# libraz/mygram-db

Hardware: AMD Instinct MI355X
Metric: queries/sec + p50 latency, 10M-doc bigram index, batch=1024 3-term AND (higher is better)
Workload: dtype u32 set algebra + f64 BM25

## Files before the change

mygram-db_amd/csrc/mgx_api.cpp:

```cpp
#include <hip/hip_runtime.h>

#include <dlfcn.h>
#include <pthread.h>

#include <algorithm>
#include <atomic>
#include <chrono>
#include <cmath>
#include <condition_variable>
#include <map>
#include <cstdio>
#include <cstdlib>
#include <cstring>
#include <memory>
#include <mutex>
#include <string>
#include <thread>
#include <tuple>
#include <unordered_map>
#include <vector>

#include "../../include/mygram_gpu.h"
#include "mgx_compile.hpp"
#include "mgx_highlight.hpp"
// ... 1481 lines not shown
    bool on() const { return !plan.queries.empty(); }
    bool requested(uint32_t qi) const { return on() && of_query[qi] >= 0; }
  };
  Documents doc;
  bool fetched = false;
  std::vector<mgx_query_result> h_results;
  std::vector<uint32_t> h_docs;
  std::vector<double> h_scores;
  bool executed = false;
  hipStream_t last_stream = nullptr;
  bool timing = false;
  std::vector<std::pair<hipEvent_t, hipEvent_t>> events;
  uint64_t list_bytes = 0;
};

namespace mgx {

constexpr int kSections = 7;
static std::atomic<uint64_t> g_section_us[kSections];
static const char* const kSectionNames[kSections] = {"queries+leaves", "routes", "table uploads", "result blocks",
                                                      "items", "launch order", "descriptors+items"};
struct SectionTimer {
  static bool On() {
    static const bool on = std::getenv("MGX_TRACE_HOST") != nullptr;
    return on;
  }
  std::chrono::steady_clock::time_point t;
  SectionTimer() { if (On()) t = std::chrono::steady_clock::now(); }
  void Mark(int section) {
    if (!On()) return;
    const auto now = std::chrono::steady_clock::now();
    g_section_us[section] += std::chrono::duration_cast<std::chrono::nanoseconds>(now - t).count();
    t = now;
  }
};

using Group = mgx_batch::Group;
using RouteLaunch = mgx_batch::RouteLaunch;

enum class Route : uint8_t {
  kBlock,
  kWave,
  kWaveLists,
  kFast,
  kCand,
  kMerge,
};

static bool EnvZero(const char* name) { return std::getenv(name) && atoi(std::getenv(name)) == 0; }
struct PathSwitches {
  const bool wave = std::getenv("MGX_FORCE_BLOCK_KERNEL") == nullptr;
  const bool fast = wave && !EnvZero("MGX_FAST_PATH"), cand = wave && !EnvZero("MGX_CAND");
  const bool merge = wave && !EnvZero("MGX_MERGE");
};

struct GroupPlan {
  GroupPlan(uint32_t n_, uint32_t mode)
      : n(n_), score_mode(mode == kModeScore), df_mode(mode == kModeTextDf), page_mode(mode == kModeDocPage) {}
  const uint32_t n;
  const bool score_mode, df_mode, page_mode;
  std::vector<DevQuery> dq;
  std::vector<DevLeaf> leaves;
  std::vector<uint32_t> prog;
  std::vector<DevScoreTerm> score;
  std::vector<uint32_t> expl;
  uint32_t max_limit = 1, max_needed = 1;
  std::vector<Route> route;
  std::vector<DevFastQuery> fastq;
  std::vector<uint64_t> wave_tables;
  std::vector<uint32_t> cand_driver;
  std::vector<DevItem> items;
  std::vector<uint32_t> list_begin, item_begin;
  std::vector<DevItem> block, wave, wave_lists, fast[kFastMaxScore], cand, merge;
  std::vector<uint8_t> has_seed;
};

static int LayOutQueries(mgx_batch* b, Group& g, const std::vector<QuerySpec>& specs, GroupPlan& p) {
  std::vector<DevLeaf>& leaves = p.leaves;
  std::vector<uint32_t>& expl = p.expl;
  p.dq.resize(p.n);
  uint32_t max_leaves = 0, max_lds_leaves = 0, max_score = 0, max_stack = 0, max_instr = 0, max_cap = 64;
  for (uint32_t i = 0; i < p.n; ++i) {
    const QuerySpec& s = specs[g.qids[i]];
    DevQuery& q = p.dq[i];
    std::memset(&q, 0, sizeof(q));
    q.leaf_begin = static_cast<uint32_t>(leaves.size());
    q.n_leaves = static_cast<uint32_t>(s.leaves.size());
    q.prog_begin = static_cast<uint32_t>(p.prog.size());
    q.n_instr = static_cast<uint32_t>(s.prog.size());
    q.score_begin = static_cast<uint32_t>(p.score.size());
    q.n_score = static_cast<uint32_t>(s.score.size());
    q.mode = s.mode;
    q.limit = s.limit;
    q.offset = s.offset;
    q.needed = static_cast<uint32_t>(std::min<uint64_t>(static_cast<uint64_t>(s.offset) + s.limit, 0xFFFFFFFFull));
    uint32_t cap = 64;
    if (s.mode == kModeScore)
      while (cap < q.needed && cap < (1u << 30)) cap <<= 1;
    q.cap = cap;
    q.descending = s.reverse;
    q.stack_depth = s.stack_depth;
    q.out_slot = i;
    q.pat_off = s.pat_off;
    q.pat_len = s.pat_len;
    q.vt_begin = s.vt_begin;
    q.vt_count = static_cast<uint32_t>(s.verify_patterns.size());
    q.fz_distance = s.fz_distance;
    q.vp_begin = s.vp_begin;
    q.k1 = s.k1;
    q.b = s.b;
    q.one_minus_b = 1.0 - s.b;
    q.k1_plus_1 = s.k1 + 1.0;
    q.avgdl_clamped = std::max(s.avgdl, 1.0);
    const uint32_t ebase = static_cast<uint32_t>(expl.size());
    uint32_t n_lds = 0;
    for (size_t li = 0; li < s.leaves.size(); ++li) {
      DevLeaf lf = s.leaves[li];
      if (lf.kind == kLeafExplicit) lf.a += ebase;
      bool resident = lf.kind == kLeafList || lf.kind == kLeafExplicit;
      for (const DevScoreTerm& st : s.score) resident = resident || st.leaf == li;
      lf.lds = resident ? n_lds++ : kNoRow;
      leaves.push_back(lf);
    }
    if (n_lds > kMaxLdsLeaves)
      return Fail(MGX_ERR_NOT_IMPLEMENTED,
                  "query " + std::to_string(g.qids[i]) + ": more than 64 sorted-list / scored operands in one query");
    max_lds_leaves = std::max(max_lds_leaves, n_lds);
    p.prog.insert(p.prog.end(), s.prog.begin(), s.prog.end());
    p.score.insert(p.score.end(), s.score.begin(), s.score.end());
    expl.insert(expl.end(), s.explicit_ids.begin(), s.explicit_ids.end());
    while (expl.size() % 4) expl.push_back(0xFFFFFFFFu);
    max_leaves = std::max(max_leaves, q.n_leaves);
    max_score = std::max(max_score, q.n_score);
    max_stack = std::max(max_stack, q.stack_depth);
    max_instr = std::max(max_instr, q.n_instr);
    max_cap = std::max(max_cap, q.cap);
    p.max_limit = std::max(p.max_limit, q.limit);
    p.max_needed = std::max(p.max_needed, q.needed);
    if (!p.df_mode) b->list_bytes += 4 * s.list_postings;
  }
  g.plan = PlanLds(max_leaves, max_lds_leaves, max_score, max_stack, max_instr, max_cap, p.score_mode || p.df_mode);
  return MGX_OK;
}

static bool ResolveFast(mgx_index* idx, const uint64_t* cond_arena, const QuerySpec& s, const DevQuery& q, DevFastQuery* out) {
  DevFastQuery& f = *out;
  for (uint32_t ins : s.prog) {
    const uint32_t op = ins >> 24, arg = ins & 0xFFFFFFu;
    if (op == kOpCount) {
      if (f.n_ops == 0) return false;
      f.ops[f.n_ops - 1].code |= arg << 8;
      continue;
    }
    const DevLeaf& lf = s.leaves[arg];
    if (f.n_ops == static_cast<uint32_t>(kFastMaxOps) || (op == kOpLoad) != (f.n_ops == 0)) return false;
    FastOp o{};
    uint64_t stride = 0;
    if (lf.kind == kLeafGramBitmap) {
      o.base = reinterpret_cast<uint64_t>(idx->dev.gram_bitmaps + static_cast<uint64_t>(lf.b) * idx->dev.gb_row_stride);
      stride = idx->dev.gb_tile_stride * 8;
    } else if (lf.kind == kLeafFilterBitmap) {
      o.base = static_cast<uint64_t>(lf.b) * idx->dev.fb_row_stride * 8;
      stride = idx->dev.fb_tile_stride * 8;
      o.code |= 16u;
    } else if (lf.kind == kLeafCondBitmap) {
      o.base = reinterpret_cast<uint64_t>(cond_arena + static_cast<uint64_t>(lf.b) * idx->dev.fb_row_stride);
      stride = idx->dev.fb_tile_stride * 8;
    } else {
      return false;
    }
    if (stride > 0xFFFFFFFFull) return false;
    o.tile_stride = static_cast<uint32_t>(stride);
    o.code |= (op == kOpLoad || op == kOpOr) ? kFastOr : op == kOpAnd ? kFastAnd : kFastAndNot;
    f.ops[f.n_ops++] = o;
  }
  if (f.n_ops == 0) return false;
  for (size_t t = 0; t < s.score.size(); ++t) {
    const DevLeaf& lf = s.leaves[s.score[t].leaf];
    if (lf.kind != kLeafGramBitmap) return false;
    FastScore& fs = f.score[t];
    fs.nib = reinterpret_cast<uint64_t>(idx->dev.tfnib + static_cast<uint64_t>(lf.b) * idx->dev.nib_row_stride);
    fs.idf = s.score[t].idf;
    fs.gram = lf.a;
    fs.skip_row = lf.row;
  }
  if (s.reverse != 0) {
    double step = 0.0;
    f.blockmax = GetBlockMax(idx, s.k1, s.b, s.avgdl, &step, &f.blockmax_fine);
    if (f.blockmax) {
      f.bm_tile_stride = idx->n_bitmap_rows * 256u;
      f.bmf_tile_stride = idx->n_fine_rows * 1024u;
      double idf_max = 0.0;
      for (size_t t = 0; t < s.score.size(); ++t) idf_max = std::max(idf_max, s.score[t].idf);
      const double wunit = idf_max > 0.0 ? idf_max * (1.0 + 0x1p-40) / 255.0 : 1.0;
      f.bm_inv_unit = 1.0 / (wunit * step);
      f.bm_wpack = f.bm_w4 = f.bm_cint = 0;
      for (size_t t = 0; t < s.score.size(); ++t) {
        const uint32_t w = static_cast<uint32_t>(std::min(255.0, std::ceil(s.score[t].idf / wunit)));
        if (t < 4) f.bm_wpack |= w << (8 * t); else f.bm_w4 = w;
      }
      for (size_t t = 0; t < s.score.size(); ++t) {
        const DevLeaf& lf = s.leaves[s.score[t].leaf];
        FastScore& fs = f.score[t];
        const uint32_t frow = f.blockmax_fine ? idx->h_fine_map[lf.b] : kNoRow;
        fs.bm_mode = frow != kNoRow ? 2u : 1u;
        fs.bm_off = frow != kNoRow ? frow * 1024u : lf.b * 256u;
      }
    }
  }
  f.n_score = static_cast<uint32_t>(s.score.size());
  f.needed = q.needed;
  f.cap = q.cap;
  f.descending = q.descending;
  f.k1 = q.k1;
  f.b = q.b;
  f.one_minus_b = q.one_minus_b;
  f.k1_plus_1 = q.k1_plus_1;
  f.avgdl_clamped = q.avgdl_clamped;
  return true;
}

static void RouteCandMerge(mgx_batch* b, Group& g, const std::vector<QuerySpec>& specs, const PathSwitches& sw,
                           GroupPlan& p) {
  static const uint64_t kMaxPerTile = std::getenv("MGX_CAND_MAX_PER_TILE") ? static_cast<uint64_t>(atoll(std::getenv("MGX_CAND_MAX_PER_TILE"))) : 64ull;
  const mgx_index* idx = b->idx;
  for (uint32_t i = 0; sw.cand && i < p.n; ++i) {
    const QuerySpec& s = specs[g.qids[i]];
    if (p.route[i] == Route::kFast || !s.flat || s.prog.empty()) continue;
    if (p.score_mode && (!s.fast_score_ok || s.score.empty())) continue;
    bool ok = true, counted = false;
    uint32_t driver = kNoLeaf;
    uint64_t best = ~0ull, longest_list = 0;
    for (size_t pc = 0; ok && pc < s.prog.size(); ++pc) {
      const uint32_t op = s.prog[pc] >> 24, arg = s.prog[pc] & 0xFFFFFFu;
      if (op == kOpCount) {
        counted = true;
        continue;
      }
      if ((op == kOpLoad) != (pc == 0) || (op != kOpLoad && op != kOpAnd && op != kOpAndNot)) { ok = false; break; }
      const DevLeaf& lf = s.leaves[arg];
      if (lf.kind != kLeafList && lf.kind != kLeafGramBitmap && !IsFilterKind(lf.kind)) { ok = false; break; }
      if (lf.kind == kLeafList) longest_list = std::max<uint64_t>(longest_list, idx->h_offsets[lf.a + 1] - idx->h_offsets[lf.a]);
      if (op == kOpAndNot || IsFilterKind(lf.kind) || counted) continue;
      const uint64_t sz = idx->h_offsets[lf.a + 1] - idx->h_offsets[lf.a];
      if (sz < best) {
        best = sz;
        driver = arg;
      }
    }
    if (!ok || driver == kNoLeaf || s.leaves[driver].kind != kLeafList) continue;
    for (uint32_t ins : s.prog)
      if ((ins >> 24) == kOpAndNot && (ins & 0xFFFFFFu) == driver) ok = false;
    if (p.score_mode)
      for (const DevScoreTerm& st : s.score)
        ok = ok && st.leaf != kNoLeaf && (s.leaves[st.leaf].kind == kLeafList || s.leaves[st.leaf].kind == kLeafGramBitmap);
    if (!ok) continue;
    DevQuery& q = p.dq[i];
    const bool long_probe = longest_list > 8 * kMaxPerTile * idx->dev.n_tiles;
    if (best > kMaxPerTile * idx->dev.n_tiles || long_probe) {
      uint32_t staged = 0;
      for (size_t li = 0; li < s.leaves.size(); ++li) staged += li != driver ? 1u : 0u;
      if (!p.score_mode || !sw.merge || staged > kMergeMaxOps || q.cap > 256) continue;
      q.pat_off = driver;
      p.route[i] = Route::kMerge;
      g.merge_leaves = std::max(g.merge_leaves, q.n_leaves);
      g.merge_instr = std::max(g.merge_instr, q.n_instr);
      g.merge_ops = std::max(g.merge_ops, staged);
      g.merge_cap = std::max(g.merge_cap, q.cap);
      continue;
    }
    if (p.cand_driver.empty()) p.cand_driver.assign(p.n, kNoLeaf);
    p.cand_driver[i] = driver;
    p.route[i] = Route::kCand;
    g.cand_leaves = std::max(g.cand_leaves, q.n_leaves);
    g.cand_instr = std::max(g.cand_instr, q.n_instr);
    g.cand_cap = std::max(g.cand_cap, q.cap);
  }
  if (CandLdsBytes(g.cand_leaves, g.cand_instr, p.score_mode ? g.cand_cap : 0) > 150 * 1024) {
    for (Route& r : p.route)
      if (r == Route::kCand) r = Route::kBlock;
    p.cand_driver.clear();
  }
  if (MergeLdsBytes(g.merge_leaves, g.merge_instr, g.merge_ops, g.merge_cap) > 150 * 1024)
    for (Route& r : p.route)
      if (r == Route::kMerge) r = Route::kBlock;
}

static int ChooseRoutes(mgx_batch* b, Group& g, const std::vector<QuerySpec>& specs, const PathSwitches& sw,
                        GroupPlan& p) {
  mgx_index* idx = b->idx;
  p.route.assign(p.n, Route::kBlock);
  if (p.score_mode) {
    uint32_t fcap = 64;
    bool have_params = false;
    double pk1 = 0, pb = 0, pavg = 0;
    for (uint32_t i = 0; sw.fast && i < p.n; ++i) {
      const QuerySpec& s = specs[g.qids[i]];
      if (!s.flat || !s.fast_score_ok || s.score.empty() || s.score.size() > static_cast<size_t>(kFastMaxScore)) continue;
      if (p.dq[i].cap > 128) continue;
      if (have_params && (Bits(s.k1) != Bits(pk1) || Bits(s.b) != Bits(pb) || Bits(s.avgdl) != Bits(pavg))) continue;
      DevFastQuery f{};
      if (!ResolveFast(idx, b->cond_arena, s, p.dq[i], &f)) continue;
      if (!have_params) {
        pk1 = s.k1;
        pb = s.b;
        pavg = s.avgdl;
        have_params = true;
      }
      if (p.fastq.empty()) p.fastq.resize(p.n);
      p.fastq[i] = f;
      p.route[i] = Route::kFast;
      fcap = std::max(fcap, f.cap);
    }
    if (have_params) {
      const double* ktab = GetLengthNormTable(idx, pk1, pb, pavg);
      g.fplan = PlanFast(fcap, ktab);
      if (ktab == nullptr || g.fplan.bytes > 64 * 1024)
        for (Route& r : p.route) r = Route::kBlock;
    }

    uint32_t wl = 0, wsc = 0, wi = 0, wc = 64;
    for (uint32_t i = 0; i < p.n; ++i) {
      if (p.route[i] == Route::kFast) continue;
      const QuerySpec& s = specs[g.qids[i]];
      bool ok = sw.wave && s.wave_ok;
      for (const DevScoreTerm& st : s.score)
        ok = ok && (s.leaves[st.leaf].kind == kLeafGramBitmap || s.leaves[st.leaf].kind == kLeafList);
      if (!ok) continue;
      uint64_t tabs[kWaveScoreSlots] = {0, 0, 0};
      for (size_t t = 0; ok && t < s.score.size(); ++t) {
        const DevLeaf& lf = s.leaves[s.score[t].leaf];
        const uint32_t key = lf.kind == kLeafGramBitmap ? lf.b : 0x80000000u | lf.a;
        tabs[t] = GetContributionTable(idx, key, s.score[t].idf, s.k1, s.b, s.avgdl);
        ok = tabs[t] != 0;
      }
      if (!ok) continue;
      if (p.wave_tables.empty()) p.wave_tables.assign(static_cast<size_t>(p.n) * kWaveScoreSlots, 0);
      for (int t = 0; t < kWaveScoreSlots; ++t) p.wave_tables[static_cast<size_t>(i) * kWaveScoreSlots + t] = tabs[t];
      bool lists = false;
      for (const DevLeaf& lf : s.leaves) lists = lists || lf.kind == kLeafList || lf.kind == kLeafExplicit;
      p.route[i] = lists ? Route::kWaveLists : Route::kWave;
      wl = std::max<uint32_t>(wl, p.dq[i].n_leaves);
      wsc = std::max<uint32_t>(wsc, p.dq[i].n_score);
      wi = std::max<uint32_t>(wi, p.dq[i].n_instr);
      wc = std::max<uint32_t>(wc, p.dq[i].cap);
    }
    g.wplan = PlanWave(wl, wsc, wi, wc, idx->dev.max_doc_len, false);
    g.wplan_lists = PlanWave(wl, wsc, wi, wc, idx->dev.max_doc_len, true);
    if (g.wplan_lists.bytes > 160 * 1024)
      for (Route& r : p.route)
        if (r != Route::kFast) r = Route::kBlock;
  }
  if (p.page_mode || p.df_mode) {
    uint32_t wl = 1, wi = 1;
    bool has_list = false;
// ... 274 lines not shown
    d.wave_tables = g.d_tables.as<uint64_t>();
  }
  if (!p.fastq.empty()) MGX_HIP(Upload(g.d_fast_queries, p.fastq.data(), p.fastq.size()));
  d.fast_queries = g.d_fast_queries.as<DevFastQuery>();
  d.dev_index = b->idx->d_dev_index.as<DevIndex>();
  d.cond_bitmaps = b->cond_arena;
  for (int t = 0; t < kFastMaxScore; ++t) MGX_HIP(MakeRoute(g.fast[t], d, p.fast[t]));
  MGX_HIP(MakeRoute(g.wave_lists, d, p.wave_lists));
  MGX_HIP(MakeRoute(g.cand, d, p.cand));
  MGX_HIP(MakeRoute(g.merge, d, p.merge));
  if (p.page_mode && !p.cand.empty()) {
    std::vector<uint8_t> skip(n, 0);
    for (uint32_t i = 0; i < n; ++i) skip[i] = p.route[i] == Route::kCand ? 1 : 0;
    MGX_HIP(Upload(g.d_cand_skip, skip.data(), skip.size()));
  }
  MGX_HIP(MakeRoute(g.block, d, p.block));
  MGX_HIP(MakeRoute(g.wave, d, p.wave));
  MGX_HIP(Upload(g.d_list_begin, p.list_begin.data(), p.list_begin.size()));
  if (p.page_mode) {
    std::vector<DevItem> pw, pb;
    for (uint32_t i = 0; i < n; ++i)
      if (p.route[i] != Route::kCand && !specs[g.qids[i]].fz_op)
        (p.route[i] == Route::kWave ? pw : pb).push_back(DevItem{i, 0, 0, 0});
    g.n_page_fz = 0;
    for (uint32_t i = 0; i < n; ++i)
      if (specs[g.qids[i]].fz_op) {
        pb.push_back(DevItem{i, 0, 0, 0});
        ++g.n_page_fz;
      }
    MGX_HIP(MakeRoute(g.page_wave, d, pw));
    MGX_HIP(MakeRoute(g.page_block, d, pb));
  }
  return MGX_OK;
}

static int UploadGroup(mgx_batch* b, Group& g, uint32_t mode, const std::vector<QuerySpec>& specs) {
  GroupPlan p(static_cast<uint32_t>(g.qids.size()), mode);
  if (p.n == 0) return MGX_OK;
  const PathSwitches sw;
  SectionTimer sec;
  if (const int rc = LayOutQueries(b, g, specs, p)) return rc;
  sec.Mark(0);
  if (const int rc = ChooseRoutes(b, g, specs, sw, p)) return rc;
  sec.Mark(1);
  if (const int rc = UploadTables(b, g, p, sec)) return rc;
  sec.Mark(3);
  CutItems(b, g, specs, p);
  sec.Mark(4);
  if (const int rc = ScheduleItems(b, g, specs, p)) return rc;
  sec.Mark(5);
  if (const int rc = UploadItems(b, g, specs, p)) return rc;
  sec.Mark(6);
  if (std::getenv("MGX_VERBOSE")) {
    size_t fast_queries = 0;
    for (Route r : p.route) fast_queries += r == Route::kFast ? 1 : 0;
    fprintf(stderr,
            "[mgx] %s group: %u queries; fast path %zu items (%zu queries, lds %u B, ring %u), wave kernel %zu items "
            "(lds %u B, lists %zu), block kernel %zu items (lds %u B), candidate-driven %zu queries, list merge %zu "
            "items\n",
            p.score_mode ? "score" : p.page_mode ? "docid-page" : p.df_mode ? "df" : "bitmap", p.n,
            p.fast[0].size() + p.fast[1].size() + p.fast[2].size() + p.fast[3].size() + p.fast[4].size(), fast_queries,
            g.fplan.bytes, g.fplan.ring, p.wave.size() + p.wave_lists.size(), g.wplan.bytes, p.wave_lists.size(),
            p.block.size(), g.plan.bytes, p.cand.size(), p.merge.size());
  }
  return MGX_OK;
}

static CompileView ViewOf(const mgx_index* idx) {
  CompileView v;
  v.offsets = idx->h_offsets.data();
  v.skip_row = idx->h_skip_row.data();
  v.bm_row = idx->h_bm_row.data();
  v.n_grams = idx->n_grams;
  v.n_docs = idx->dev.n_docs;
  v.first_doc_id = idx->dev.first_doc_id;
  v.has_text = idx->dev.text != nullptr;
  v.can_score = idx->can_score;
  v.n_filter_rows = idx->n_filter_rows;
  v.n_filter_columns = idx->n_filter_columns.load(std::memory_order_acquire);
  v.live_row = idx->live_row.load(std::memory_order_relaxed);
  v.bitmaps_clean = idx->bitmaps_clean.load(std::memory_order_relaxed);
  static const bool pk_general = [] {
    const char* e = std::getenv("MGX_PK_SORT_GENERAL");
    return e != nullptr && e[0] != '\0' && e[0] != '0';
  }();
  v.pk_docid_order = !pk_general && !idx->has_doc_map.load(std::memory_order_acquire) && idx->pk_monotone.load(std::memory_order_acquire) &&
                     idx->pk_shortcut.load(std::memory_order_relaxed);
  return v;
}

static int CompileRange(const CompileView& view, const mgx_query* queries, std::vector<QuerySpec>* specs, uint32_t a, uint32_t b) {
  for (uint32_t i = a; i < b; ++i) {
    (*specs)[i].Clear();
    if (const int rc = CompileQuery(view, queries[i], &(*specs)[i])) return Fail(rc, "query " + std::to_string(i) + ": " + g_last_error);
  }
  return MGX_OK;
}

struct CompilePool {
  std::mutex mu, gate;
  std::condition_variable cv_work, cv_done;
  std::vector<std::thread> helpers;
  const CompileView* view = nullptr;
  const mgx_query* queries = nullptr;
  std::vector<QuerySpec>* specs = nullptr;
  uint32_t next = 0, end = 0, pending = 0;
  int rc = MGX_OK;
  std::string error;
  bool stop = false;
  static constexpr uint32_t kChunk = 64;

  void Run(std::unique_lock<std::mutex>& lock) {
    while (next < end) {
      const uint32_t a = next, b = std::min(end, a + kChunk);
// ... 2840 lines not shown
```

mygram-db_amd/csrc/mgx_internal.hpp:

```cpp
#pragma once

#include <cstdint>

namespace mgx {

constexpr int kBlock = 256;
constexpr int kTileShift = 14;
constexpr uint32_t kTileDocs = 1u << kTileShift;
constexpr int kWordsPerTile = kTileDocs / 64;
constexpr int kMaxTilesPerItem = 64;
constexpr uint32_t kNoRow = 0xFFFFFFFFu;
constexpr uint32_t kMaxLeaves = 192;
constexpr uint32_t kMaxLdsLeaves = 64;
constexpr uint32_t kMaxScoreTerms = 64;
constexpr uint32_t kMaxNeeded = 1024;
constexpr uint32_t kMergeMaxOps = 6;
constexpr uint32_t kMatchBuf = 2048;

enum LeafKind : uint32_t {
  kLeafList = 0,
  kLeafGramBitmap = 1,
  kLeafFilterBitmap = 2,
  kLeafRange = 3,
  kLeafExplicit = 4,
// ... 73 lines not shown
  kModeDocCount = 3,
  kModeDocPage = 4,
};
constexpr uint32_t kMaxDocPage = 16384;

struct DevQuery {
  uint32_t leaf_begin, n_leaves;
  uint32_t prog_begin, n_instr;
  uint32_t score_begin, n_score;
  uint32_t mode;
  uint32_t cap;
  uint32_t needed;
  uint32_t limit, offset;
  uint32_t descending;
  uint32_t stack_depth;
  uint32_t out_slot;
  uint32_t pat_off, pat_len;
  uint32_t vt_begin, vt_count;
  uint32_t fz_distance;
  uint32_t vp_begin;
  double k1, b, one_minus_b, k1_plus_1, avgdl_clamped;
};

constexpr uint32_t kFzBuf = 2048;
constexpr uint32_t kFzLdsBytes = kWordsPerTile * 8 + 16 + kFzBuf * 2;

struct DevIndex {
  const uint64_t* offsets;
  const uint32_t* docids;
  const uint8_t* tf;
  const uint64_t* tf_ovf_pos;
  const uint32_t* tf_ovf_val;
  uint32_t n_tf_ovf;
  const uint32_t* doc_len;
  const uint8_t* dl8;
  const uint8_t* tfnib;
  uint64_t nib_row_stride;
  const uint32_t* skip_row;
  const uint32_t* tile_off;
  const uint64_t* gram_bitmaps;
  uint64_t gb_tile_stride, gb_row_stride;
  const uint64_t* filter_bitmaps;
  uint64_t fb_tile_stride, fb_row_stride;
  const uint8_t* text;
  const uint64_t* text_off;
  uint32_t first_doc_id;
  uint32_t n_docs;
  uint32_t n_tiles;
  uint32_t max_doc_len;
};

constexpr int kFastMaxOps = 8;
constexpr int kFastMaxScore = 5;
constexpr uint32_t kFastPoolTf = 14;
#ifndef MGX_FWAVES
#define MGX_FWAVES 8
#endif
constexpr int kFastBlock = 64 * MGX_FWAVES;
constexpr int kFastWaves = kFastBlock / 64;

enum FastOpKind : uint32_t { kFastOr = 0, kFastAnd = 1, kFastAndNot = 2 };
struct FastOp {
  uint64_t base;
  uint32_t tile_stride;
  uint32_t code;
};
struct FastScore {
  uint64_t nib;
  double idf;
  uint32_t gram, skip_row;
  uint32_t bm_mode, bm_off;
};
struct DevFastQuery {
  uint32_t n_ops, n_score, needed, cap;
  uint32_t descending, pad0;
  uint32_t pad1, pad1b;
  uint32_t bm_wpack, bm_w4;
  uint32_t bm_cint, pad2;
  double bm_inv_unit;
  double k1, b, one_minus_b, k1_plus_1, avgdl_clamped;
  const uint8_t* blockmax;
  const uint8_t* blockmax_fine;
  uint32_t bm_tile_stride, bmf_tile_stride;
  FastOp ops[kFastMaxOps];
  FastScore score[kFastMaxScore];
};
static_assert(sizeof(DevFastQuery) % 8 == 0, "DevFastQuery is read with scalar loads");

struct FastPlan {
  uint32_t ring;
  uint32_t max_cap;
  uint32_t bytes, pad;
  const double* ktab;
};
struct TableJob {
  double idf, k1, b, avgdl;
  uint32_t slot, pad;
};
FastPlan PlanFast(uint32_t max_cap, const double* ktab);
uint32_t FastTableDl(uint32_t max_doc_len);

struct DevItem {
  uint32_t query, tile_begin, n_tiles, list;
};

struct DevCondition {
  uint64_t literal;
  double eq_epsilon;
  uint32_t op, null_matches, never_matches;
  uint32_t row;
};
struct DevCondGroup {
  const uint64_t* values;
  const uint8_t* is_null;
  uint32_t value_class, cond_begin, cond_end, pad;
};
static_assert(sizeof(DevCondition) % 8 == 0 && sizeof(DevCondGroup) % 8 == 0, "read with scalar loads");
constexpr uint32_t kCondWordsPerWave = 8;
constexpr uint32_t kCondBlockWords = kCondWordsPerWave * (kBlock / 64);

struct DevBatch {
  const DevItem* items;
  uint32_t n_items;
  const DevQuery* queries;
  const DevLeaf* leaves;
  const uint32_t* prog;
  const DevScoreTerm* score_terms;
  const uint32_t* explicit_pool;
// ... 82 lines not shown
```

mygram-db_amd/csrc/mgx_kernels.hip:

```cpp
#include <hip/hip_runtime.h>

#include <algorithm>
#include <cstdlib>

#include "mgx_fuzzy.hpp"
#include "mgx_internal.hpp"
#include "mgx_launch.hpp"

namespace mgx {

#ifdef MGX_ABLATION
#define MGX_ABLATE(bt, bit) (((bt).debug_skip & (bit)) != 0)
#else
#define MGX_ABLATE(bt, bit) false
#endif


__device__ __forceinline__ int lane_id() { return threadIdx.x & 63; }

__device__ __forceinline__ uint32_t wave_uniform(uint32_t v) { return __builtin_amdgcn_readfirstlane(v); }
__device__ __forceinline__ float wave_uniform(float v) {
  return __uint_as_float(__builtin_amdgcn_readfirstlane(__float_as_uint(v)));
}
__device__ __forceinline__ uint64_t wave_uniform(uint64_t v) {
// ... 1634 lines not shown
      }
    }
    if (tid == 0) bt.cand_n[it.list] = min(total, q.needed);
  }
}

__global__ __launch_bounds__(kWaveBlock, 6) void wave_score_kernel(DevIndex ix, DevBatch bt, WavePlan plan) {
  wave_score_body(ix, bt, plan);
}
__global__ __launch_bounds__(kWaveBlock, 6) void wave_score_lists_kernel(DevIndex ix, DevBatch bt, WavePlan plan) {
  wave_score_body(ix, bt, plan);
}


#ifndef MGX_FPL
#define MGX_FPL 4
#endif
constexpr int kFastPerLane = MGX_FPL;
constexpr uint32_t kFastRound = 64 * kFastPerLane;
constexpr uint32_t kFastPairs = 320;

struct FastOffsets {
  uint32_t ktab, pairs, ring, tk_keys, tk_docs, misc, total;
};
__host__ __device__ inline FastOffsets carve_fast(const FastPlan& p) {
  FastOffsets o;
  uint32_t at = 0;
  o.ktab = at;     at += 256 * 8;
  o.pairs = at;    at += kFastWaves * kFastPairs * 8;
  o.ring = at;     at += kFastWaves * p.ring * 4;
  o.tk_keys = at;  at += kFastWaves * 2 * p.max_cap * 8;
  o.tk_docs = at;  at += kFastWaves * 2 * p.max_cap * 4;
  o.misc = at;     at += 64;
  o.total = at;
  return o;
}
uint32_t FastTableDl(uint32_t max_doc_len) {
  const uint32_t t = max_doc_len + 1 < kTableDlMax ? max_doc_len + 1 : kTableDlMax;
  return (t + 1u) & ~1u;
}
FastPlan PlanFast(uint32_t max_cap, const double* ktab) {
  FastPlan p{};
  p.ring = kFastRound + 128;
  p.max_cap = max_cap;
  p.ktab = ktab;
  p.bytes = carve_fast(p).total;
  return p;
}

typedef uint32_t u32x4 __attribute__((ext_vector_type(4)));
typedef const u32x4 __attribute__((address_space(1)))* gptr_u4;
typedef const uint32_t __attribute__((address_space(1)))* gptr_u1;
typedef const DevFastQuery __attribute__((address_space(4)))* FastQueryPtr;

__device__ __noinline__ uint32_t fast_exact_tf(const DevIndex* ix, uint32_t gram, uint32_t row, uint32_t slot) {
  return exact_tf(*ix, gram, row, slot);
}

template <int T>
__device__ __forceinline__ void fast_load_blockmax(const FastQueryPtr fq, uint32_t tile, uint32_t lane, u32x4 (&raw)[T]) {
  const uint64_t bm = reinterpret_cast<uint64_t>(fq->blockmax), bmf = reinterpret_cast<uint64_t>(fq->blockmax_fine);
  const uint32_t st = fq->bm_tile_stride, stf = fq->bmf_tile_stride;
#pragma unroll
  for (int i = 0; i < T; ++i) {
    const bool fine = fq->score[i].bm_mode == 2u;
    const uint64_t row = (fine ? bmf : bm) + static_cast<uint64_t>(tile) * (fine ? stf : st) + fq->score[i].bm_off;
    const uint32_t off = fine ? lane << 4 : (lane >> 2) << 4;
    raw[i] = *reinterpret_cast<gptr_u4>(row + off);
  }
}

template <int T>
__device__ __forceinline__ uint32_t fast_quarter_mask(const FastQueryPtr fq, uint32_t lane, const u32x4 (&raw)[T],
                                                      uint64_t bound) {
  const uint32_t tint = static_cast<uint32_t>(
      fmin(floor(key_score(bound, true) * fq->bm_inv_unit * (1.0 - 0x1p-30)), 4294967040.0));
  const uint32_t wpack = fq->bm_wpack, w4 = fq->bm_w4, cint = fq->bm_cint;
  uint32_t bmw[T][4];
#pragma unroll
  for (int i = 0; i < T; ++i) {
    bmw[i][0] = raw[i].x;
    bmw[i][1] = raw[i].y;
    bmw[i][2] = raw[i].z;
    bmw[i][3] = raw[i].w;
    const uint32_t mode = fq->score[i].bm_mode;
    if (mode == 1u) {
      const uint32_t l3 = lane & 3u;
      const uint32_t c = l3 == 0u ? raw[i].x : l3 == 1u ? raw[i].y : l3 == 2u ? raw[i].z : raw[i].w;
      bmw[i][0] = __builtin_amdgcn_perm(0u, c, 0x00000000u);
      bmw[i][1] = __builtin_amdgcn_perm(0u, c, 0x01010101u);
      bmw[i][2] = __builtin_amdgcn_perm(0u, c, 0x02020202u);
      bmw[i][3] = __builtin_amdgcn_perm(0u, c, 0x03030303u);
    } else if (mode != 2u) {
      bmw[i][0] = bmw[i][1] = bmw[i][2] = bmw[i][3] = 0;
    }
  }
  uint32_t mk = 0;
#pragma unroll
  for (int k = 0; k < 4; ++k) {
    const uint32_t t0 = bmw[0][k], t1 = T > 1 ? bmw[T > 1 ? 1 : 0][k] : 0u, t2 = T > 2 ? bmw[T > 2 ? 2 : 0][k] : 0u,
                   t3 = T > 3 ? bmw[T > 3 ? 3 : 0][k] : 0u;
    const uint32_t lo01 = __builtin_amdgcn_perm(t1, t0, 0x05010400u), hi01 = __builtin_amdgcn_perm(t1, t0, 0x07030602u);
    const uint32_t lo23 = T > 2 ? __builtin_amdgcn_perm(t3, t2, 0x05010400u) : 0u;
    const uint32_t hi23 = T > 2 ? __builtin_amdgcn_perm(t3, t2, 0x07030602u) : 0u;
    uint32_t qb[4];
    qb[0] = __builtin_amdgcn_perm(lo23, lo01, 0x05040100u);
    qb[1] = __builtin_amdgcn_perm(lo23, lo01, 0x07060302u);
    qb[2] = __builtin_amdgcn_perm(hi23, hi01, 0x05040100u);
    qb[3] = __builtin_amdgcn_perm(hi23, hi01, 0x07060302u);
#pragma unroll
    for (int j = 0; j < 4; ++j) {
      uint32_t ub = __builtin_amdgcn_udot4(qb[j], wpack, cint, false);
      if (T > 4) ub += w4 * ((bmw[T > 4 ? 4 : 0][k] >> (8 * j)) & 255u);
      if (ub >= tint) mk |= 1u << (4 * k + j);
    }
  }
  return mk;
}

template <int T>
__device__ __noinline__ uint32_t fast_remask(const FastQueryPtr fq, uint32_t tile, uint32_t lane, uint64_t bound) {
  u32x4 raw[T];
  fast_load_blockmax<T>(fq, tile, lane, raw);
  return fast_quarter_mask<T>(fq, lane, raw, bound);
}

template <int T>
__device__ __forceinline__ void bitmap_score_body(const DevIndex& ix, const DevBatch& bt, const FastPlan& plan,
                                                  const FastQueryPtr fq, const DevItem it) {
  extern __shared__ __attribute__((aligned(16))) unsigned char smem[];
  const FastOffsets fo = carve_fast(plan);
  const uint32_t tid = threadIdx.x, lane = tid & 63u, wave = wave_uniform(tid >> 6);
  double* const ktab = reinterpret_cast<double*>(smem + fo.ktab);
  uint32_t* const ring = reinterpret_cast<uint32_t*>(smem + fo.ring) + wave * plan.ring;
  uint2* const pairs = reinterpret_cast<uint2*>(smem + fo.pairs) + wave * kFastPairs;
  uint32_t* const misc = reinterpret_cast<uint32_t*>(smem + fo.misc);
  const uint32_t n_ops = fq->n_ops;
  const bool desc = fq->descending != 0;
  const uint32_t tile_begin = it.tile_begin;
  const uint32_t tile_end = min(tile_begin + it.n_tiles, ix.n_tiles);

  if (tid < 256) ktab[tid] = plan.ktab[tid];

  WaveTopK tk;
  tk.cap = fq->cap;
  tk.needed = fq->needed;
  tk.lds_sort = true;
  tk.keys = reinterpret_cast<uint64_t*>(smem + fo.tk_keys) + static_cast<size_t>(wave) * 2 * fq->cap;
  tk.docs = reinterpret_cast<uint32_t*>(smem + fo.tk_docs) + static_cast<size_t>(wave) * 2 * fq->cap;
  tk.have = 0;
  tk.pend = 0;
  tk.bound_key = 0;
  tk.bound_doc = 0;
  tk.gbound_ptr = bt.bounds ? bt.bounds + it.query : nullptr;
  tk.gbound = 0;
  for (uint32_t i = lane; i < 2 * tk.cap; i += 64) {
    tk.keys[i] = 0;
    tk.docs[i] = 0;
  }
  __syncthreads();

  __amdgpu_buffer_rsrc_t nib_rsrc[T];
  double idf[T];
#pragma unroll
  for (int i = 0; i < T; ++i) {
    nib_rsrc[i] = __builtin_amdgcn_make_buffer_rsrc(reinterpret_cast<void*>(fq->score[i].nib), 0,
                                                    static_cast<int>((ix.n_docs + 1u) >> 1), 0x00020000);
    idf[i] = fq->score[i].idf;
  }
  const __amdgpu_buffer_rsrc_t dl_rsrc = __builtin_amdgcn_make_buffer_rsrc(
      const_cast<uint8_t*>(ix.dl8), 0, static_cast<int>(ix.n_docs), 0x00020000);
  const double k1_plus_1 = fq->k1_plus_1;
  const bool prune = fq->blockmax != 0;

  uint32_t cnt0 = 0, cnt1 = 0, cnt2 = 0, cnt3 = 0, cnt_res = 0;
  uint32_t pend = 0;
  uint32_t np = 0;

  auto score_round = [&](uint32_t g0, uint32_t n) {
    uint32_t slot[kFastPerLane], dli[kFastPerLane], nb[kFastPerLane][T];
#pragma unroll
    for (int m = 0; m < kFastPerLane; ++m) {
// ... 10 lines not shown
    for (int m = 0; m < kFastPerLane; ++m) {
      if (static_cast<uint32_t>(m) * 64u >= n) break;
      uint32_t sl = slot[0], dl = dli[0], nbm[T];
#pragma unroll
      for (int i = 0; i < T; ++i) nbm[i] = nb[0][i];
#pragma unroll
      for (int mm = 1; mm < kFastPerLane; ++mm) {
        if (m == mm) {
          sl = slot[mm];
          dl = dli[mm];
#pragma unroll
          for (int i = 0; i < T; ++i) nbm[i] = nb[mm][i];
        }
      }
      const bool valid = static_cast<uint32_t>(m) * 64u + lane < n;
      double kd = ktab[dl];
      const uint32_t sh = (sl & 1u) << 2;
      uint32_t tf[T], mx = 0;
#pragma unroll
      for (int i = 0; i < T; ++i) {
        tf[i] = (nbm[i] >> sh) & 15u;
        mx = max(mx, tf[i]);
      }
      if (__ballot(valid && (mx == 15u || dl == 255u)) != 0) {
#pragma unroll
        for (int i = 0; i < T; ++i)
          if (valid && tf[i] == 15u) tf[i] = fast_exact_tf(bt.dev_index, fq->score[i].gram, fq->score[i].skip_row, sl);
        if (valid && dl == 255u) {
          const double dld = static_cast<double>(ix.doc_len[sl]);
          kd = fq->k1 * (fq->one_minus_b + fq->b * dld / fq->avgdl_clamped);
        }
      }
      double score = 0.0;
#pragma unroll
      for (int i = 0; i < T; ++i) {
        const double tfd = static_cast<double>(tf[i]);
        const double c = tf[i] != 0u ? idf[i] * (tfd * k1_plus_1) / (tfd + kd) : 0.0;
        score = i == 0 ? c : score + c;
      }
      const uint32_t doc = ix.first_doc_id + sl;
      wave_topk_offer(tk, valid, score_key(score, desc), desc ? doc : ~doc);
    }
  };

  auto load_half = [&](uint32_t o, uint32_t tile, uint32_t h) {
    const uint64_t op_base = fq->ops[o].base;
    const uint32_t op_code = fq->ops[o].code, op_stride = fq->ops[o].tile_stride;
    const uint64_t base = op_base + ((op_code & 16u) ? reinterpret_cast<uint64_t>(ix.filter_bitmaps) : 0ull) +
                          static_cast<uint64_t>(tile) * op_stride;
    const gptr_u4 p = reinterpret_cast<gptr_u4>(base) + lane * 2 + h;
    return p[0];
  };

  for (uint32_t tile = tile_begin + wave;; tile += kFastWaves) {
    const bool flush = tile >= tile_end;
    uint32_t a[8] = {0, 0, 0, 0, 0, 0, 0, 0};
    uint64_t bound = 0;
    if (!flush) {
      wave_topk_refresh_gbound(tk);
      uint32_t qmask = 0xFFFFu;
      if (prune) {
        bound = tk.gbound;
        if (tk.have >= tk.needed && tk.bound_key > bound) bound = tk.bound_key;
      }
      u32x4 raw[T];
#pragma unroll
      for (int i = 0; i < T; ++i) raw[i] = u32x4{0u, 0u, 0u, 0u};
      if (prune) fast_load_blockmax<T>(fq, tile, lane, raw);
      auto combine = [&](int h, uint32_t o, const u32x4 w) {
        const uint32_t code = fq->ops[o].code;
        const uint32_t x[4] = {w.x, w.y, w.z, w.w};
        const uint32_t kind = wave_uniform(code & 15u);
        if (kind == kFastAnd) {
#pragma unroll
          for (int j = 0; j < 4; ++j) a[h * 4 + j] &= x[j];
        } else if (kind == kFastOr) {
#pragma unroll
          for (int j = 0; j < 4; ++j) a[h * 4 + j] |= x[j];
        } else {
#pragma unroll
          for (int j = 0; j < 4; ++j) a[h * 4 + j] &= ~x[j];
        }
        const uint32_t cmask = wave_uniform(code >> 8);
        if (cmask) {
          uint32_t pc = 0;
#pragma unroll
          for (int j = 0; j < 4; ++j) pc += __popc(a[h * 4 + j]);
          if (cmask & 1u) cnt0 += pc;
          if (cmask & 2u) cnt1 += pc;
          if (cmask & 4u) cnt2 += pc;
          if (cmask & 8u) cnt3 += pc;
        }
      };
      const uint32_t o1 = min(1u, n_ops - 1u), o2 = min(2u, n_ops - 1u);
      u32x4 w[2][3];
#pragma unroll
      for (int h = 0; h < 2; ++h) {
        w[h][0] = load_half(0, tile, h);
        w[h][1] = load_half(o1, tile, h);
        w[h][2] = load_half(o2, tile, h);
      }
      if (bound != 0) qmask = fast_quarter_mask<T>(fq, lane, raw, bound);
#pragma unroll
      for (int h = 0; h < 2; ++h) {
        combine(h, 0, w[h][0]);
        if (n_ops > 1u) combine(h, 1, w[h][1]);
        if (n_ops > 2u) combine(h, 2, w[h][2]);
        for (uint32_t o = 3; o < n_ops; ++o) combine(h, o, load_half(o, tile, h));
      }
#pragma unroll
      for (int j = 0; j < 8; ++j) cnt_res += __popc(a[j]);
      if (qmask != 0xFFFFu && !MGX_ABLATE(bt, 128u)) {
#pragma unroll
        for (int j = 0; j < 8; ++j) {
          const uint32_t m2 = qmask >> (2 * j);
          a[j] &= ((m2 & 1u) ? 0x0000FFFFu : 0u) | ((m2 & 2u) ? 0xFFFF0000u : 0u);
        }
      }
      if (MGX_ABLATE(bt, 2u)) {
#pragma unroll
        for (int j = 0; j < 8; ++j) a[j] = 0;
      }
    }

    const uint32_t slot0 = tile * kTileDocs + lane * 256u;
    bool scored = false;
#pragma nounroll
    for (uint32_t part = 0; part < 2u; ++part) {
      if (!flush) {
#ifndef MGX_NO_REMASK
        if (part != 0u && scored && prune) {
          wave_topk_refresh_gbound(tk);
          uint64_t nb = tk.gbound;
          if (tk.have >= tk.needed && tk.bound_key > nb) nb = tk.bound_key;
          if (nb > bound) {
            bound = nb;
            const uint32_t qm = fast_remask<T>(fq, tile, lane, nb);
#pragma unroll
            for (int j = 4; j < 8; ++j) {
              const uint32_t m2 = qm >> (2 * j);
              a[j] &= ((m2 & 1u) ? 0x0000FFFFu : 0u) | ((m2 & 2u) ? 0xFFFF0000u : 0u);
            }
          }
        }
#endif
#pragma unroll
        for (int j = 0; j < 4; ++j) {
          const uint32_t w = part != 0u ? a[4 + j] : a[j];
          const uint64_t m = __ballot(w != 0u);
          if (m != 0) {
            if (w != 0u) {
              const uint32_t at = np + __builtin_amdgcn_mbcnt_hi(static_cast<uint32_t>(m >> 32),
                                                                 __builtin_amdgcn_mbcnt_lo(static_cast<uint32_t>(m), 0u));
              pairs[at] = make_uint2(slot0 + (part * 4u + j) * 32u, w);
            }
            np += static_cast<uint32_t>(__popcll(m));
          }
        }
      }
      for (;;) {
        if (np < 64u && !(flush && (np != 0u || pend != 0u))) break;
// ... 62 lines not shown
#pragma unroll
      for (int d = 32; d > 0; d >>= 1) x += __shfl_down(x, d, 64);
      if (lane == 0 && x) atomicAdd(&bt.counters[static_cast<uint64_t>(it.query) * 8 + s], (unsigned long long)x);
    }
  }

  wave_topk_truncate(tk);
  if (lane == 0) misc[wave] = tk.have;
  __syncthreads();
  {
    const uint64_t* all_keys = reinterpret_cast<const uint64_t*>(smem + fo.tk_keys);
    const uint32_t* all_docs = reinterpret_cast<const uint32_t*>(smem + fo.tk_docs);
    const uint32_t cap = tk.cap, needed = tk.needed;
    uint32_t have[kFastWaves];
    uint32_t total = 0;
    for (int w = 0; w < kFastWaves; ++w) {
      have[w] = min(misc[w], needed);
      total += have[w];
    }
    const uint64_t obase = static_cast<uint64_t>(it.list) * bt.cand_stride;
    for (uint32_t e = tid; e < kFastWaves * cap; e += kFastBlock) {
      const uint32_t w = e / cap, i = e % cap;
      if (i >= have[w]) continue;
      const uint64_t k = all_keys[static_cast<size_t>(w) * 2 * cap + i];
      const uint32_t d = all_docs[static_cast<size_t>(w) * 2 * cap + i];
      uint32_t rank = i;
      for (uint32_t w2 = 0; w2 < kFastWaves; ++w2) {
        if (w2 == w) continue;
        const uint64_t* kk = all_keys + static_cast<size_t>(w2) * 2 * cap;
        const uint32_t* dd = all_docs + static_cast<size_t>(w2) * 2 * cap;
        uint32_t lo = 0, hi = have[w2];
        while (lo < hi) {
          const uint32_t mid = (lo + hi) >> 1;
          if (better(kk[mid], dd[mid], k, d)) lo = mid + 1; else hi = mid;
        }
        rank += lo;
      }
      if (rank < needed) {
        bt.cand_keys[obase + rank] = k;
        bt.cand_docs[obase + rank] = d;
        if (rank == needed - 1 && tk.gbound_ptr) atomicMax(tk.gbound_ptr, static_cast<unsigned long long>(k));
      }
    }
    if (tid == 0) bt.cand_n[it.list] = min(total, needed);
  }
}

template <int T>
#ifndef MGX_FOCC
#define MGX_FOCC 6
#endif
__global__ __launch_bounds__(kFastBlock, MGX_FOCC) void bitmap_score_kernel(DevIndex ix, DevBatch bt, FastPlan plan) {
  const DevItem it = bt.items[blockIdx.x];
  bitmap_score_body<T>(ix, bt, plan,
                       reinterpret_cast<FastQueryPtr>(reinterpret_cast<uint64_t>(bt.fast_queries + it.query)), it);
}


template <bool kLists>
__device__ __forceinline__ void wave_operand_words(const DevIndex& ix, const DevBatch& bt, const DevLeaf lf,
                                                   uint32_t tile, bool active, uint64_t* scratch, uint64_t (&w)[4]) {
  const uint32_t lane = lane_id();
#pragma unroll
  for (int k = 0; k < 4; ++k) w[k] = 0;
  if (!active) return;
  if (kLists) {
    uint32_t seg_rel;
    wave_fetch_operand(ix, bt, lf, tile, static_cast<uint64_t>(ix.first_doc_id) + static_cast<uint64_t>(tile) * kTileDocs,
                       scratch, w, &seg_rel);
  } else if (lf.kind == kLeafRange) {
#pragma unroll
    for (int k = 0; k < 4; ++k) {
      const uint64_t s0 = static_cast<uint64_t>(tile) * kTileDocs + (static_cast<uint64_t>(lane) * 4 + k) * 64;
      const uint64_t ra = lf.a > s0 ? lf.a - s0 : 0, rb = lf.b > s0 ? lf.b - s0 : 0;
      const uint64_t hi_mask = rb >= 64 ? ~0ull : ((1ull << rb) - 1ull);
      const uint64_t lo_mask = ra >= 64 ? ~0ull : ((1ull << ra) - 1ull);
      w[k] = hi_mask & ~lo_mask;
    }
  } else {
    const uint64_t* rowp = lf.kind == kLeafGramBitmap
                               ? ix.gram_bitmaps + tile * ix.gb_tile_stride + lf.b * ix.gb_row_stride + lane * 4
                               : filter_rows(ix, bt.cond_bitmaps, lf.kind) + tile * ix.fb_tile_stride + lf.b * ix.fb_row_stride + lane * 4;
    const uint4 v0 = *reinterpret_cast<const uint4*>(rowp);
    const uint4 v1 = *reinterpret_cast<const uint4*>(rowp + 2);
    w[0] = (static_cast<uint64_t>(v0.y) << 32) | v0.x;
    w[1] = (static_cast<uint64_t>(v0.w) << 32) | v0.z;
    w[2] = (static_cast<uint64_t>(v1.y) << 32) | v1.x;
    w[3] = (static_cast<uint64_t>(v1.w) << 32) | v1.z;
  }
}

constexpr uint32_t kDfMatchBuf = 512;

template <bool kLists, bool kTextDf>
__global__ __launch_bounds__(kBlock) void wave_count_kernel(DevIndex ix, DevBatch bt, WavePlan plan) {
  extern __shared__ __attribute__((aligned(16))) unsigned char smem[];
  DevLeaf* const leaf = reinterpret_cast<DevLeaf*>(smem);
  uint32_t* const prog = reinterpret_cast<uint32_t*>(smem + align8(plan.max_leaves * static_cast<uint32_t>(sizeof(DevLeaf))));
  uint64_t* const scratch_all = reinterpret_cast<uint64_t*>(
      smem + align8(plan.max_leaves * static_cast<uint32_t>(sizeof(DevLeaf))) + align8(plan.max_instr * 4));
  const uint32_t tid = threadIdx.x, lane = lane_id(), wave = wave_id();
  uint64_t* const scratch = scratch_all + (kLists ? static_cast<size_t>(wave) * kWordsPerTile : 0);
  constexpr int kT = (kLists || kTextDf) ? 1 : 2;
  constexpr int kWaves = kBlock / 64;
  uint16_t* const mbuf = reinterpret_cast<uint16_t*>(scratch_all + (kLists ? kWaves * kWordsPerTile : 0)) +
                         static_cast<size_t>(wave) * kDfMatchBuf;

  const DevItem it = bt.items[blockIdx.x];
// ... 1999 lines not shown
```

Before: 1.074 million.

## Add specialized plain-AND fast path with hoisted scalar query constants

Adds a host-side classification marking score queries that are pure ANDs of gram bitmaps, each scored once and in order, as 'plain'. These queries take a templated kernel variant that hoists operand bases, strides, blockmax pointers and flags into scalar registers once per item. The variant issues the bitmap and blockmax loads directly, overlaps the global-bound atomic load with the operand loads, and unrolls the AND combine without per-op code dispatch. The goal is to cut per-tile constant-memory reloads and branching, at the cost of a second kernel specialization, more register pressure, and a slightly staler bound refresh order.

```diff
diff --git a/mygram-db_amd/csrc/mgx_api.cpp b/mygram-db_amd/csrc/mgx_api.cpp
--- a/mygram-db_amd/csrc/mgx_api.cpp
+++ b/mygram-db_amd/csrc/mgx_api.cpp
@@ -1557,6 +1557,7 @@
   const bool wave = std::getenv("MGX_FORCE_BLOCK_KERNEL") == nullptr;
   const bool fast = wave && !EnvZero("MGX_FAST_PATH"), cand = wave && !EnvZero("MGX_CAND");
   const bool merge = wave && !EnvZero("MGX_MERGE");
+  const bool plain = !EnvZero("MGX_PLAIN");
 };
 
 struct GroupPlan {
@@ -1648,8 +1649,10 @@
   return MGX_OK;
 }
 
-static bool ResolveFast(mgx_index* idx, const uint64_t* cond_arena, const QuerySpec& s, const DevQuery& q, DevFastQuery* out) {
+static bool ResolveFast(mgx_index* idx, const uint64_t* cond_arena, const QuerySpec& s, const DevQuery& q, bool allow_plain,
+                        DevFastQuery* out) {
   DevFastQuery& f = *out;
+  bool plain = allow_plain && s.score.size() <= static_cast<size_t>(kFastPlainMax);
   for (uint32_t ins : s.prog) {
     const uint32_t op = ins >> 24, arg = ins & 0xFFFFFFu;
     if (op == kOpCount) {
@@ -1677,6 +1680,8 @@
     if (stride > 0xFFFFFFFFull) return false;
     o.tile_stride = static_cast<uint32_t>(stride);
     o.code |= (op == kOpLoad || op == kOpOr) ? kFastOr : op == kOpAnd ? kFastAnd : kFastAndNot;
+    plain = plain && lf.kind == kLeafGramBitmap && (op == kOpLoad || op == kOpAnd) && f.n_ops < s.score.size() &&
+            s.score[f.n_ops].leaf == arg && stride * kFastWaves <= 0xFFFFFFFFull;
     f.ops[f.n_ops++] = o;
   }
   if (f.n_ops == 0) return false;
@@ -1714,6 +1719,9 @@
     }
   }
   f.n_score = static_cast<uint32_t>(s.score.size());
+  plain = plain && f.n_ops == f.n_score &&
+          static_cast<uint64_t>(std::max(f.bm_tile_stride, f.bmf_tile_stride)) * kFastWaves <= 0xFFFFFFFFull;
+  f.plain = plain ? 1u : 0u;
   f.needed = q.needed;
   f.cap = q.cap;
   f.descending = q.descending;
@@ -1805,7 +1813,7 @@
       if (p.dq[i].cap > 128) continue;
       if (have_params && (Bits(s.k1) != Bits(pk1) || Bits(s.b) != Bits(pb) || Bits(s.avgdl) != Bits(pavg))) continue;
       DevFastQuery f{};
-      if (!ResolveFast(idx, b->cond_arena, s, p.dq[i], &f)) continue;
+      if (!ResolveFast(idx, b->cond_arena, s, p.dq[i], sw.plain, &f)) continue;
       if (!have_params) {
         pk1 = s.k1;
         pb = s.b;
@@ -2186,14 +2194,17 @@
   if (const int rc = UploadItems(b, g, specs, p)) return rc;
   sec.Mark(6);
   if (std::getenv("MGX_VERBOSE")) {
-    size_t fast_queries = 0;
-    for (Route r : p.route) fast_queries += r == Route::kFast ? 1 : 0;
+    size_t fast_queries = 0, plain_queries = 0;
+    for (uint32_t i = 0; i < p.n; ++i) {
+      fast_queries += p.route[i] == Route::kFast ? 1 : 0;
+      plain_queries += p.route[i] == Route::kFast && p.fastq[i].plain ? 1 : 0;
+    }
     fprintf(stderr,
-            "[mgx] %s group: %u queries; fast path %zu items (%zu queries, lds %u B, ring %u), wave kernel %zu items "
+            "[mgx] %s group: %u queries; fast path %zu items (%zu queries, plain %zu, lds %u B, ring %u), wave kernel %zu items "
             "(lds %u B, lists %zu), block kernel %zu items (lds %u B), candidate-driven %zu queries, list merge %zu "
             "items\n",
             p.score_mode ? "score" : p.page_mode ? "docid-page" : p.df_mode ? "df" : "bitmap", p.n,
-            p.fast[0].size() + p.fast[1].size() + p.fast[2].size() + p.fast[3].size() + p.fast[4].size(), fast_queries,
+            p.fast[0].size() + p.fast[1].size() + p.fast[2].size() + p.fast[3].size() + p.fast[4].size(), fast_queries, plain_queries,
             g.fplan.bytes, g.fplan.ring, p.wave.size() + p.wave_lists.size(), g.wplan.bytes, p.wave_lists.size(),
             p.block.size(), g.plan.bytes, p.cand.size(), p.merge.size());
   }
diff --git a/mygram-db_amd/csrc/mgx_internal.hpp b/mygram-db_amd/csrc/mgx_internal.hpp
--- a/mygram-db_amd/csrc/mgx_internal.hpp
+++ b/mygram-db_amd/csrc/mgx_internal.hpp
@@ -149,6 +149,7 @@
 
 constexpr int kFastMaxOps = 8;
 constexpr int kFastMaxScore = 5;
+constexpr int kFastPlainMax = 3;
 constexpr uint32_t kFastPoolTf = 14;
 #ifndef MGX_FWAVES
 #define MGX_FWAVES 8
@@ -170,7 +171,7 @@
 };
 struct DevFastQuery {
   uint32_t n_ops, n_score, needed, cap;
-  uint32_t descending, pad0;
+  uint32_t descending, plain;
   uint32_t pad1, pad1b;
   uint32_t bm_wpack, bm_w4;
   uint32_t bm_cint, pad2;
diff --git a/mygram-db_amd/csrc/mgx_kernels.hip b/mygram-db_amd/csrc/mgx_kernels.hip
--- a/mygram-db_amd/csrc/mgx_kernels.hip
+++ b/mygram-db_amd/csrc/mgx_kernels.hip
@@ -1710,6 +1710,22 @@
 typedef const u32x4 __attribute__((address_space(1)))* gptr_u4;
 typedef const uint32_t __attribute__((address_space(1)))* gptr_u1;
 typedef const DevFastQuery __attribute__((address_space(4)))* FastQueryPtr;
+__device__ __forceinline__ uint32_t fast_keep(uint32_t x) {
+  asm volatile("" : "+s"(x));
+  return x;
+}
+__device__ __forceinline__ uint64_t fast_keep(uint64_t x) {
+  asm volatile("" : "+s"(x));
+  return x;
+}
+__device__ __forceinline__ double fast_keep(double x) {
+  asm volatile("" : "+s"(x));
+  return x;
+}
+__device__ __forceinline__ uint32_t fast_keep_v(uint32_t x) {
+  asm volatile("" : "+v"(x));
+  return x;
+}
 
 __device__ __noinline__ uint32_t fast_exact_tf(const DevIndex* ix, uint32_t gram, uint32_t row, uint32_t slot) {
   return exact_tf(*ix, gram, row, slot);
@@ -1729,11 +1745,27 @@
 }
 
 template <int T>
-__device__ __forceinline__ uint32_t fast_quarter_mask(const FastQueryPtr fq, uint32_t lane, const u32x4 (&raw)[T],
+struct FastBmConst {
+  double inv_unit;
+  uint32_t wpack, w4, cint, mode[T];
+};
+template <int T>
+__device__ __forceinline__ FastBmConst<T> fast_bm_const(const FastQueryPtr fq) {
+  FastBmConst<T> c;
+  c.inv_unit = fq->bm_inv_unit;
+  c.wpack = fq->bm_wpack;
+  c.w4 = fq->bm_w4;
+  c.cint = fq->bm_cint;
+#pragma unroll
+  for (int i = 0; i < T; ++i) c.mode[i] = fq->score[i].bm_mode;
+  return c;
+}
+template <int T>
+__device__ __forceinline__ uint32_t fast_quarter_mask(const FastBmConst<T>& bc, uint32_t lane, const u32x4 (&raw)[T],
                                                       uint64_t bound) {
   const uint32_t tint = static_cast<uint32_t>(
-      fmin(floor(key_score(bound, true) * fq->bm_inv_unit * (1.0 - 0x1p-30)), 4294967040.0));
-  const uint32_t wpack = fq->bm_wpack, w4 = fq->bm_w4, cint = fq->bm_cint;
+      fmin(floor(key_score(bound, true) * bc.inv_unit * (1.0 - 0x1p-30)), 4294967040.0));
+  const uint32_t wpack = bc.wpack, w4 = bc.w4, cint = bc.cint;
   uint32_t bmw[T][4];
 #pragma unroll
   for (int i = 0; i < T; ++i) {
@@ -1741,9 +1773,9 @@
     bmw[i][1] = raw[i].y;
     bmw[i][2] = raw[i].z;
     bmw[i][3] = raw[i].w;
-    const uint32_t mode = fq->score[i].bm_mode;
+    const uint32_t mode = bc.mode[i];
     if (mode == 1u) {
-      const uint32_t l3 = lane & 3u;
+      const uint32_t l3 = fast_keep_v(lane) & 3u;
       const uint32_t c = l3 == 0u ? raw[i].x : l3 == 1u ? raw[i].y : l3 == 2u ? raw[i].z : raw[i].w;
       bmw[i][0] = __builtin_amdgcn_perm(0u, c, 0x00000000u);
       bmw[i][1] = __builtin_amdgcn_perm(0u, c, 0x01010101u);
@@ -1780,12 +1812,13 @@
 __device__ __noinline__ uint32_t fast_remask(const FastQueryPtr fq, uint32_t tile, uint32_t lane, uint64_t bound) {
   u32x4 raw[T];
   fast_load_blockmax<T>(fq, tile, lane, raw);
-  return fast_quarter_mask<T>(fq, lane, raw, bound);
-}
-
-template <int T>
+  return fast_quarter_mask<T>(fast_bm_const<T>(fq), lane, raw, bound);
+}
+
+template <int T, bool kPlain>
 __device__ __forceinline__ void bitmap_score_body(const DevIndex& ix, const DevBatch& bt, const FastPlan& plan,
                                                   const FastQueryPtr fq, const DevItem it) {
+  static_assert(!kPlain || T <= kFastPlainMax, "a plain AND has at most kFastPlainMax operands");
   extern __shared__ __attribute__((aligned(16))) unsigned char smem[];
   const FastOffsets fo = carve_fast(plan);
   const uint32_t tid = threadIdx.x, lane = tid & 63u, wave = wave_uniform(tid >> 6);
@@ -1902,21 +1935,63 @@
     return p[0];
   };
 
+  constexpr int TP = kPlain ? T : 1;
+  uint64_t p_op[TP], p_bm[TP];
+  uint32_t p_op_stride = 0, p_bm_stride[TP];
+  uint32_t p_flags = 0;
+  FastBmConst<T> p_bc{};
+  if constexpr (kPlain) {
+    p_op_stride = fast_keep(fq->ops[0].tile_stride);
+    const uint64_t bm = reinterpret_cast<uint64_t>(fq->blockmax), bmf = reinterpret_cast<uint64_t>(fq->blockmax_fine);
+    const uint32_t st = fq->bm_tile_stride, stf = fq->bmf_tile_stride;
+#pragma unroll
+    for (int i = 0; i < T; ++i) {
+      p_op[i] = fast_keep(fq->ops[i].base);
+      const uint32_t mode = fq->score[i].bm_mode;
+      p_flags |= ((fq->ops[i].code >> 8) & 15u) << (4 * i) | (mode & 3u) << (12 + 2 * i);
+      const bool fine = mode == 2u;
+      p_bm[i] = fast_keep(prune ? (fine ? bmf : bm) + fq->score[i].bm_off : fq->ops[i].base);
+      p_bm_stride[i] = fast_keep(prune ? (fine ? stf : st) : fq->ops[0].tile_stride);
+    }
+    p_flags = fast_keep(p_flags);
+    p_bc.inv_unit = fast_keep(fq->bm_inv_unit);
+    p_bc.wpack = fast_keep(fq->bm_wpack);
+    p_bc.w4 = 0;
+    p_bc.cint = fast_keep(fq->bm_cint);
+  }
+
   for (uint32_t tile = tile_begin + wave;; tile += kFastWaves) {
     const bool flush = tile >= tile_end;
     uint32_t a[8] = {0, 0, 0, 0, 0, 0, 0, 0};
     uint64_t bound = 0;
     if (!flush) {
-      wave_topk_refresh_gbound(tk);
       uint32_t qmask = 0xFFFFu;
-      if (prune) {
-        bound = tk.gbound;
-        if (tk.have >= tk.needed && tk.bound_key > bound) bound = tk.bound_key;
+      auto best_bound = [&]() {
+        uint64_t bd = tk.gbound;
+        if (tk.have >= tk.needed && tk.bound_key > bd) bd = tk.bound_key;
+        return bd;
+      };
+      if constexpr (!kPlain) {
+        wave_topk_refresh_gbound(tk);
+        if (prune) bound = best_bound();
       }
       u32x4 raw[T];
-#pragma unroll
-      for (int i = 0; i < T; ++i) raw[i] = u32x4{0u, 0u, 0u, 0u};
-      if (prune) fast_load_blockmax<T>(fq, tile, lane, raw);
+      if constexpr (kPlain) {
+        const uint32_t fl = fast_keep(p_flags);
+        const uint32_t ln = fast_keep_v(lane), lane_f = ln << 4, lane_c = (ln >> 2) << 4;
+#pragma unroll
+        for (int i = 0; i < T; ++i) {
+          const uint64_t row = fast_keep(p_bm[i] + static_cast<uint64_t>(tile) * p_bm_stride[i]);
+          const uint32_t off = (fl >> (12 + 2 * i) & 3u) == 2u ? lane_f : lane_c;
+          raw[i] = *reinterpret_cast<gptr_u4>(row + static_cast<uint64_t>(off));
+        }
+      } else {
+#pragma unroll
+        for (int i = 0; i < T; ++i) raw[i] = u32x4{0u, 0u, 0u, 0u};
+        if (prune) fast_load_blockmax<T>(fq, tile, lane, raw);
+      }
+      uint64_t gfly = 0;
+      if constexpr (kPlain) gfly = __hip_atomic_load(tk.gbound_ptr, __ATOMIC_RELAXED, __HIP_MEMORY_SCOPE_AGENT);
       auto combine = [&](int h, uint32_t o, const u32x4 w) {
         const uint32_t code = fq->ops[o].code;
         const uint32_t x[4] = {w.x, w.y, w.z, w.w};
@@ -1944,19 +2019,66 @@
       };
       const uint32_t o1 = min(1u, n_ops - 1u), o2 = min(2u, n_ops - 1u);
       u32x4 w[2][3];
-#pragma unroll
-      for (int h = 0; h < 2; ++h) {
-        w[h][0] = load_half(0, tile, h);
-        w[h][1] = load_half(o1, tile, h);
-        w[h][2] = load_half(o2, tile, h);
-      }
-      if (bound != 0) qmask = fast_quarter_mask<T>(fq, lane, raw, bound);
-#pragma unroll
-      for (int h = 0; h < 2; ++h) {
-        combine(h, 0, w[h][0]);
-        if (n_ops > 1u) combine(h, 1, w[h][1]);
-        if (n_ops > 2u) combine(h, 2, w[h][2]);
-        for (uint32_t o = 3; o < n_ops; ++o) combine(h, o, load_half(o, tile, h));
+      if constexpr (kPlain) {
+        const uint64_t tile_off = static_cast<uint64_t>(tile) * p_op_stride;
+        const uint32_t voff = fast_keep_v(lane) * 32u;
+        uint64_t row[T];
+#pragma unroll
+        for (int i = 0; i < T; ++i) row[i] = fast_keep(p_op[i] + tile_off);
+#pragma unroll
+        for (int h = 0; h < 2; ++h) {
+#pragma unroll
+          for (int i = 0; i < T; ++i) w[h][i] = reinterpret_cast<gptr_u4>(row[i] + static_cast<uint64_t>(voff))[h];
+        }
+      } else {
+#pragma unroll
+        for (int h = 0; h < 2; ++h) {
+          w[h][0] = load_half(0, tile, h);
+          w[h][1] = load_half(o1, tile, h);
+          w[h][2] = load_half(o2, tile, h);
+        }
+      }
+      if constexpr (kPlain) {
+        const uint64_t g = wave_uniform(gfly);
+        if (g > tk.gbound) tk.gbound = g;
+        if (prune) bound = best_bound();
+      }
+      if constexpr (kPlain) {
+        const uint32_t fl = fast_keep(p_flags);
+        if (bound != 0) {
+          FastBmConst<T> bc = p_bc;
+#pragma unroll
+          for (int i = 0; i < T; ++i) bc.mode[i] = fl >> (12 + 2 * i) & 3u;
+          qmask = fast_quarter_mask<T>(bc, lane, raw, bound);
+        }
+#pragma unroll
+        for (int h = 0; h < 2; ++h) {
+#pragma unroll
+          for (int i = 0; i < T; ++i) {
+            const uint32_t x[4] = {w[h][i].x, w[h][i].y, w[h][i].z, w[h][i].w};
+#pragma unroll
+            for (int j = 0; j < 4; ++j) a[h * 4 + j] = i == 0 ? x[j] : a[h * 4 + j] & x[j];
+            const uint32_t cmask = fl >> (4 * i) & 15u;
+            if (cmask) {
+              uint32_t pc = 0;
+#pragma unroll
+              for (int j = 0; j < 4; ++j) pc += __popc(a[h * 4 + j]);
+              if (cmask & 1u) cnt0 += pc;
+              if (cmask & 2u) cnt1 += pc;
+              if (cmask & 4u) cnt2 += pc;
+              if (cmask & 8u) cnt3 += pc;
+            }
+          }
+        }
+      } else {
+        if (bound != 0) qmask = fast_quarter_mask<T>(fast_bm_const<T>(fq), lane, raw, bound);
+#pragma unroll
+        for (int h = 0; h < 2; ++h) {
+          combine(h, 0, w[h][0]);
+          if (n_ops > 1u) combine(h, 1, w[h][1]);
+          if (n_ops > 2u) combine(h, 2, w[h][2]);
+          for (uint32_t o = 3; o < n_ops; ++o) combine(h, o, load_half(o, tile, h));
+        }
       }
 #pragma unroll
       for (int j = 0; j < 8; ++j) cnt_res += __popc(a[j]);
@@ -2125,8 +2247,14 @@
 #endif
 __global__ __launch_bounds__(kFastBlock, MGX_FOCC) void bitmap_score_kernel(DevIndex ix, DevBatch bt, FastPlan plan) {
   const DevItem it = bt.items[blockIdx.x];
-  bitmap_score_body<T>(ix, bt, plan,
-                       reinterpret_cast<FastQueryPtr>(reinterpret_cast<uint64_t>(bt.fast_queries + it.query)), it);
+  const FastQueryPtr fq = reinterpret_cast<FastQueryPtr>(reinterpret_cast<uint64_t>(bt.fast_queries + it.query));
+  if constexpr (T <= kFastPlainMax) {
+    if (fq->plain != 0) {
+      bitmap_score_body<T, true>(ix, bt, plan, fq, it);
+      return;
+    }
+  }
+  bitmap_score_body<T, false>(ix, bt, plan, fq, it);
 }
 
 
```

Result: slower. 1.052 million (-2.0%).
